# ahmad12hamdan99/CarMPC

Hardware: NVIDIA B200
Metric: terminal-set samples/s (higher is better)
Workload: dtype f64

## Files before the change

### carmpc_b200/_capi.py

```python
from __future__ import annotations

import ctypes
import os

from . import build as _build


class CarmpcError(RuntimeError):
    """A C-ABI call returned a negative status."""


class QPOpts(ctypes.Structure):
    _fields_ = [("rho", ctypes.c_double), ("alpha", ctypes.c_double), ("eps_abs", ctypes.c_double),
                ("eps_rel", ctypes.c_double), ("eps_prim_inf", ctypes.c_double),
                ("max_iter", ctypes.c_int32), ("check_every", ctypes.c_int32),
                ("scaling_iters", ctypes.c_int32), ("polish", ctypes.c_int32)]


class DisturbanceModel(ctypes.Structure):
    _fields_ = [("Bd", ctypes.c_double * 4), ("Cd", ctypes.c_double * 3), ("L1", ctypes.c_double * 12),
                ("L2", ctypes.c_double * 3), ("Bd_plant", ctypes.c_double * 4), ("Cd_plant", ctypes.c_double * 3)]


class LoopNoiseParams(ctypes.Structure):
    _fields_ = [("seed", ctypes.c_uint64), ("first_run", ctypes.c_int64), ("Lw", ctypes.c_double * 16),
                ("Lv", ctypes.c_double * 16)]


_vp, _dp, _i64, _i32 = ctypes.c_void_p, ctypes.c_void_p, ctypes.c_int64, ctypes.c_int

SIGNATURES = {
    "carmpc_last_error": (ctypes.c_char_p, []),
    "carmpc_version": (ctypes.c_char_p, []),
    "carmpc_destroy": (None, [_vp]),
    "carmpc_polytope_create": (_i32, [_dp, _i32, ctypes.POINTER(_vp)]),
    "carmpc_membership_bitset": (_i32, [_vp, _dp, _dp, _dp, _dp, _i64, _vp, _vp, _i32, _vp]),
    "carmpc_polytope_tune": (_i32, [_vp, _dp, _dp, _dp, _dp, _i64, _vp]),
    "carmpc_membership_grid": (_i32, [_vp, _dp, ctypes.POINTER(ctypes.c_int32), ctypes.POINTER(ctypes.c_int32),
                                      _vp, _vp, _vp]),
    "carmpc_membership_bitset_host": (_i32, [_vp, _dp, _dp, _dp, _dp, _i64, _vp, ctypes.POINTER(_i64), _i32]),
    "carmpc_rollout_create": (_i32, [_dp, _dp, _dp, _i32, _dp, _dp, _i32, _dp, _i32, _i32, ctypes.POINTER(_vp)]),
    "carmpc_rollout_bitset": (_i32, [_vp, _dp, _dp, _dp, _dp, _i64, _vp, _vp, _vp, _vp]),
    "carmpc_rollout_bitset_host": (_i32, [_vp, _dp, _dp, _dp, _dp, _i64, _vp, _vp, ctypes.POINTER(_i64)]),
    "carmpc_rollout_get_rows": (_i32, [_vp, _dp, _i32]),
    "carmpc_rollout_reduce_screen": (_i32, [_vp, ctypes.POINTER(ctypes.c_int32), _i32, ctypes.POINTER(ctypes.c_int32), _dp, _i32]),
    "carmpc_scan_staging": (_i32, [_vp, _i32, _i32, _i32]),
    "carmpc_shard_create": (_i32, [_i32, _i32, _i64, ctypes.POINTER(_vp)]),
    "carmpc_shard_export": (_i32, [_vp, _vp]),
    "carmpc_shard_connect": (_i32, [_vp, _vp]),
    "carmpc_shard_connect_local": (_i32, [_vp, ctypes.POINTER(_vp)]),
    "carmpc_membership_bitset_sharded": (_i32, [_vp, _vp, _dp, _dp, _dp, _dp, _i64, _i64, _i64, _i32, _vp, _i32, _vp]),
    "carmpc_rollout_bitset_sharded": (_i32, [_vp, _vp, _dp, _dp, _dp, _dp, _i64, _i64, _i64, _vp, _i32, _vp]),
# ... 73 lines not shown
```

### carmpc_b200/batch.py

```python
from __future__ import annotations

import ctypes
from dataclasses import dataclass
from typing import Optional

import numpy as np

from . import _capi
from ._capi import CarmpcError, check


def _torch():
    import torch
    return torch


def _f64(a) -> np.ndarray:
    return np.ascontiguousarray(a, dtype=np.float64)


def _stream_ptr(stream=None):
    torch = _torch()
    s = torch.cuda.current_stream() if stream is None else stream
    return ctypes.c_void_p(s.cuda_stream)
# ... 11 lines not shown
    def close(self):
        if getattr(self, "_h", None) is not None and self._h:
            self._lib.carmpc_destroy(self._h)
            self._h = ctypes.c_void_p()

    def __del__(self):
        try:
            self.close()
        except Exception:
            pass


class _ScanTuning:
    def set_staging(self, threads_per_cta: int = 256, ring_slots: int = 3, tiles_per_slot: int = 1) -> None:
        check(self._lib.carmpc_scan_staging(self._h, int(threads_per_cta), int(ring_slots), int(tiles_per_slot)))


def _check_soa(x, y, psi, v):
    torch = _torch()
    n = x.numel()
    for t in (x, y, psi, v):
        if not (t.is_cuda and t.dtype == torch.float64 and t.is_contiguous() and t.numel() == n):
            raise ValueError("x, y, psi, v must be contiguous float64 CUDA tensors of equal length")
    return n


class TerminalSetEvaluator(_Handle, _ScanTuning):

    def __init__(self, A: np.ndarray, b: Optional[np.ndarray] = None):
        super().__init__()
# ... 12 lines not shown
    def contains_bits(self, x, y, psi, v, mode: int = 1, bits=None, count=None, stream=None):
        torch = _torch()
        n = _check_soa(x, y, psi, v)
        if bits is None:
            bits = torch.empty((n + 31) // 32, dtype=torch.int32, device=x.device)
        if count is None:
            count = torch.empty(1, dtype=torch.int64, device=x.device)
        check(self._lib.carmpc_membership_bitset(self._h, x.data_ptr(), y.data_ptr(), psi.data_ptr(), v.data_ptr(),
                                                 n, bits.data_ptr(), count.data_ptr(), mode, _stream_ptr(stream)))
        return bits, count

    def tune(self, x, y, psi, v, stream=None) -> None:
        n = _check_soa(x, y, psi, v)
        check(self._lib.carmpc_polytope_tune(self._h, x.data_ptr(), y.data_ptr(), psi.data_ptr(), v.data_ptr(), n,
                                             _stream_ptr(stream)))

    def contains_grid_bits(self, axes, axis_to_state=(0, 1, 2, 3), bits=None, count=None, stream=None):
        torch = _torch()
        axes = [_f64(a).ravel() for a in axes]
        dims = (ctypes.c_int32 * 4)(*[len(a) for a in axes])
        a2s = (ctypes.c_int32 * 4)(*axis_to_state)
        n = int(np.prod([len(a) for a in axes]))
        cat = np.ascontiguousarray(np.concatenate(axes))
        if bits is None:
            bits = torch.empty((n + 31) // 32, dtype=torch.int32, device="cuda")
        if count is None:
            count = torch.empty(1, dtype=torch.int64, device="cuda")
        check(self._lib.carmpc_membership_grid(self._h, _capi.ptr(cat), dims, a2s, bits.data_ptr(), count.data_ptr(),
                                               _stream_ptr(stream)))
        return bits, count
# ... 453 lines not shown
```

### carmpc_b200/csrc/membership.cu

```cuda
#include <math.h>
#include <stdlib.h>

#include <algorithm>
#include <vector>

#include "common.cuh"
#include "shard.cuh"

namespace carmpc {

constexpr int kMaxRows = 512;
constexpr int kThreads = 256;
constexpr int kNS = 4;
constexpr int kChunk = kThreads * kNS;

struct __align__(16) RowF32 {
    float na0, na1, na2, na3;
    float b, pad0, pad1, pad2;
};

struct Staging {
    int threads = 128, stages = 2, tps = 1;
};

// ... 38 lines not shown
        }
        return CARMPC_OK;
    }
    ~HostStage() {
        for (int i = 0; i < 2; ++i) {
            cudaFree(d_coord[i]);
            cudaFree(d_bits[i]);
            cudaFree(d_first[i]);
            if (streams[i]) cudaStreamDestroy(streams[i]);
        }
        cudaFree(d_count);
        cudaFree(d_work);
    }
};

struct Polytope : HandleBase {
    int rows = 0;
    double* d_rows = nullptr;
    RowF32* d_rows32 = nullptr;
    float beta0 = 0.f, beta1 = 0.f;
    HostStage stage;
    std::vector<double> h_rows;
    bool tuned = false;
    Staging staging;
    unsigned long long* d_work = nullptr;
    double* d_axes = nullptr;
    double* h_axes = nullptr;
    ~Polytope() override {
        cudaFree(d_rows);
        cudaFree(d_rows32);
        cudaFree(d_axes);
        cudaFreeHost(h_axes);
        cudaFree(d_work);
    }
};

struct Rollout : HandleBase {
    int s = 0, rin = 0, k_steps = 0, input_mode = 0;
    double* d_data = nullptr;
    RowF32* d_rows32 = nullptr;
    int rows_padded = 0, rows32 = 0;
    float beta0 = 0.f, beta1 = 0.f;
    float in0 = 0.f, in1 = 0.f;
    std::vector<double> h_rows64;
    std::vector<RowF32> h_rows32;
// ... 419 lines not shown
        for (int d = 0; d < kMaxPeers; ++d)
            if (d < sink.n) sink.dst[d][w0] = acc;
        group = __shfl_sync(0xffffffffu, pg, 0);
    }
    block_count<THREADS>(members, count);
    if (tid == 0) {
        __threadfence();
        if (atomicAdd(work + 1, 1ull) == (unsigned long long)gridDim.x - 1ull) {
            work[0] = 0ull;
            work[1] = 0ull;
            __threadfence();
        }
    }
}

struct GridDesc {
    int32_t dims[4];
    int32_t state_of_axis[4];
    int32_t offset[4];
};

__global__ void __launch_bounds__(kThreads, 4)
membership_grid_kernel(const double* __restrict__ g_rows, const RowF32* __restrict__ g_rows32, int rows, int rows_padded,
                       const ScreenConst sc, const double* __restrict__ g_axes, GridDesc gd, int64_t n,
                       uint32_t* __restrict__ bits, unsigned long long* __restrict__ count) {
    extern __shared__ __align__(16) unsigned char smem_raw[];
    double* s_rows = reinterpret_cast<double*>(smem_raw);
    RowF32* s_rows32 = reinterpret_cast<RowF32*>(s_rows + ((rows * 5 + 1) & ~1));
    double* s_axes = reinterpret_cast<double*>(s_rows32 + rows_padded);
    const int axes_len = gd.offset[3] + gd.dims[3];
// ... 205 lines not shown
    dev &= 63;
    if (per_sm_cached[dev] <= 0 || smem_cached[dev] != smem) {
        CARMPC_CUDA(cudaFuncSetAttribute(kernel, cudaFuncAttributeMaxDynamicSharedMemorySize, (int)smem));
        int per_sm = 0;
        CARMPC_CUDA(cudaOccupancyMaxActiveBlocksPerMultiprocessor(&per_sm, kernel, THREADS, smem));
        per_sm_cached[dev] = per_sm > 0 ? per_sm : 1;
        smem_cached[dev] = smem;
    }
    const int64_t n_units = (n_groups + THREADS / 32 - 1) / (THREADS / 32);
    kernel<<<grid_blocks(n_units, per_sm_cached[dev]), THREADS, smem, st>>>(d_exact, d_rows32, es, rows_padded, sc, x, y, p, v,
                                                                      n_groups, sink, count, work);
    CARMPC_CUDA(cudaGetLastError());
    return CARMPC_OK;
}

template <int KIND>
static int launch_scan(const double* d_exact, const RowF32* d_rows32, const ExactSpec es, int rows_padded,
                       const ScreenConst sc, const double* x, const double* y, const double* p, const double* v,
                       int64_t n, BitSink sink, unsigned long long* count, unsigned long long* work, int mode, const Staging& geo,
                       cudaStream_t st) {
    if (n == 0) return CARMPC_OK;
    const bool vec = ((reinterpret_cast<uintptr_t>(x) | reinterpret_cast<uintptr_t>(y) |
                       reinterpret_cast<uintptr_t>(p) | reinterpret_cast<uintptr_t>(v)) & 15) == 0;
    if (vec && mode == 1 && n >= 64 * (int64_t)kChunk) {
        const int64_t n_groups = n / kGroup;
        const size_t smem = scan_tma_smem(es.len, rows_padded, geo);
        int rc = CARMPC_ERR_UNSUPPORTED;
#define TMA_CASE(T, S, P)                                                                                              \
        if (geo.threads == T && geo.stages == S && geo.tps == P)                                                           \
            rc = launch_tma<KIND, T, S, P>(d_exact, d_rows32, es, rows_padded, sc, x, y, p, v, n_groups, sink, count, work, smem, st)
        TMA_CASE(256, 3, 1); TMA_CASE(128, 3, 1); TMA_CASE(128, 4, 1); TMA_CASE(128, 2, 2);
        TMA_CASE(128, 3, 2); TMA_CASE(256, 2, 1); TMA_CASE(128, 2, 1); TMA_CASE(256, 2, 2);
#undef TMA_CASE
        if (rc == CARMPC_ERR_UNSUPPORTED) set_error("membership scan: staging geometry %d/%d/%d is not built", geo.threads, geo.stages, geo.tps);
        if (rc != CARMPC_OK) return rc;
        const int64_t done = n_groups * kGroup;
        if (done == n) return CARMPC_OK;
        x += done; y += done; p += done; v += done; n -= done;
        sink = offset_sink(sink, n_groups);
    }
    const size_t smem = scan_smem(es.len, rows_padded);
    const int64_t n_chunks = (n + kChunk - 1) / kChunk;
#define LAUNCH(M, V)                                                                                              \
    do {                                                                                                          \
        int per_sm = 0;                                                                                           \
        CARMPC_CUDA(cudaOccupancyMaxActiveBlocksPerMultiprocessor(&per_sm, membership_kernel<M, V, KIND>, kThreads, smem)); \
        const int blocks = grid_blocks(n_chunks, per_sm > 0 ? per_sm : 1);                                        \
        membership_kernel<M, V, KIND><<<blocks, kThreads, smem, st>>>(d_exact, d_rows32, es, rows_padded, sc, x, y, p, v, \
// ... 3 lines not shown
        if (vec) LAUNCH(0, true); else LAUNCH(0, false);
    } else {
        if (vec) LAUNCH(1, true); else LAUNCH(1, false);
    }
#undef LAUNCH
    CARMPC_CUDA(cudaGetLastError());
    return CARMPC_OK;
}

static int launch_membership(Polytope* P, const double* x, const double* y, const double* p, const double* v,
                             int64_t n, const BitSink& sink, unsigned long long* count, unsigned long long* work, int mode,
                             cudaStream_t st) {
    ExactSpec es{};
    es.len = P->rows * 5;
    es.rows = P->rows;
    return launch_scan<0>(P->d_rows, P->d_rows32, es, pad_rows(P->rows), screen_const(P), x, y, p, v, n, sink, count, work, mode,
                          P->staging, st);
}

static int launch_rollout(Rollout* R, const double* x, const double* y, const double* p, const double* v, int64_t n,
                          const BitSink& sink, int32_t* first, unsigned long long* count, unsigned long long* work, cudaStream_t st) {
    if (n == 0) return CARMPC_OK;
    if (first == nullptr && R->d_rows32 != nullptr) {
        ExactSpec es{};
        es.len = 20 + 5 * R->s + 5 * R->rin;
        es.s = R->s; es.rin = R->rin; es.k_steps = R->k_steps; es.input_mode = R->input_mode;
        ScreenConst sc;
        sc.beta0 = R->beta0; sc.beta1 = R->beta1; sc.in0 = R->in0; sc.in1 = R->in1;
        return launch_scan<1>(R->d_data, R->d_rows32, es, R->rows_padded, sc, x, y, p, v, n, sink, count, work, 1, R->staging, st);
    }
// ... 104 lines not shown
        if (best < 0 || cnt[best] == 0) break;
        used[best] = 1;
        order.push_back(best);
        size_t w = 0;
        for (unsigned long long m : alive) if (!((m >> best) & 1ull)) alive[w++] = m;
        alive.resize(w);
    }
    for (int r = 0; r < rows; ++r) if (!used[r]) order.push_back(r);
    std::vector<double> sorted(5 * rows);
    for (int i = 0; i < rows; ++i)
        for (int k = 0; k < 5; ++k) sorted[5 * i + k] = P->h_rows[5 * order[i] + k];
    P->h_rows.swap(sorted);
    return upload_rows(P, st);
}

__global__ void __launch_bounds__(256)
pilot32_kernel(const RowF32* __restrict__ g_rows32, int rows, int words, const double* __restrict__ gx,
               const double* __restrict__ gy, const double* __restrict__ gp, const double* __restrict__ gv, int64_t n,
               int64_t stride, int n_sub, unsigned long long* __restrict__ masks) {
    const int k = blockIdx.x * blockDim.x + threadIdx.x;
    if (k >= n_sub) return;
    const int64_t i = (int64_t)k * stride;
    unsigned long long* out = masks + (size_t)k * words;
    for (int w = 0; w < words; ++w) out[w] = 0ull;
    if (i >= n) return;
    const float x = (float)gx[i], y = (float)gy[i], p = (float)gp[i], v = (float)gv[i];
    for (int r = 0; r < rows; ++r) {
        const RowF32 q = g_rows32[r];
        const float m = fmaf(q.na3, v, fmaf(q.na2, p, fmaf(q.na1, y, fmaf(q.na0, x, q.b))));
        if (!(m >= 0.f)) out[r >> 6] |= 1ull << (r & 63);
// ... 98 lines not shown
    }
    const double u8 = 8.0 * 5.9604644775390625e-08, tiny = 1.401298464324817e-45;
    const double b0 = u8 * bmax * 1.000001 + l1max * tiny + 1e-37, b1 = u8 * l1max * 1.000001 + 1e-37;
    if (faithful && b0 < 1e30 && b1 < 1e30) {
        P->beta0 = nextafterf((float)b0, INFINITY);
        P->beta1 = nextafterf((float)b1, INFINITY);
    } else {
        P->beta0 = P->beta1 = INFINITY;
    }
    P->h_rows = sorted;
    h_Ab = sorted.data();
    auto fail = [&](int code) { delete P; return code; };
    if (cudaMalloc(&P->d_rows, sizeof(double) * 5 * (rows > 0 ? rows : 1)) != cudaSuccess ||
        cudaMalloc(&P->d_rows32, sizeof(RowF32) * r32.size()) != cudaSuccess ||
        cudaMalloc(&P->d_work, sizeof(unsigned long long) * 2) != cudaSuccess ||
        cudaMemset(P->d_work, 0, sizeof(unsigned long long) * 2) != cudaSuccess) {
        set_error("carmpc_polytope_create: cudaMalloc failed: %s", cudaGetErrorString(cudaGetLastError()));
        return fail(CARMPC_ERR_CUDA);
    }
    if (rows > 0) {
        if (cudaMemcpy(P->d_rows, h_Ab, sizeof(double) * 5 * rows, cudaMemcpyHostToDevice) != cudaSuccess ||
            cudaMemcpy(P->d_rows32, r32.data(), sizeof(RowF32) * r32.size(), cudaMemcpyHostToDevice) != cudaSuccess) {
            set_error("carmpc_polytope_create: cudaMemcpy failed: %s", cudaGetErrorString(cudaGetLastError()));
            return fail(CARMPC_ERR_CUDA);
        }
    }
    *handle = P;
    return CARMPC_OK;
}

int carmpc_membership_bitset(void* polytope, const double* d_x, const double* d_y, const double* d_psi,
                             const double* d_v, int64_t n, uint32_t* d_bits, int64_t* d_count, int mode,
                             void* stream) {
    Polytope* P = check_handle<Polytope>(polytope, kPolytope);
    CARMPC_REQUIRE(P != nullptr, "not a polytope handle");
    CARMPC_REQUIRE(n >= 0, "n");
    CARMPC_REQUIRE(mode == 0 || mode == 1, "mode must be 0 or 1");
    if (n == 0) {
        if (d_count) CARMPC_CUDA(cudaMemsetAsync(d_count, 0, sizeof(int64_t), (cudaStream_t)stream));
        return CARMPC_OK;
    }
    CARMPC_REQUIRE(d_x && d_y && d_psi && d_v && d_bits, "null device pointer");
    cudaStream_t st = (cudaStream_t)stream;
    if (!P->tuned && n >= ((int64_t)1 << 20)) {
        const int rc = tune_row_order(P, d_x, d_y, d_psi, d_v, n, st);
        if (rc != CARMPC_OK) return rc;
    }
    if (d_count) CARMPC_CUDA(cudaMemsetAsync(d_count, 0, sizeof(int64_t), st));
    return launch_membership(P, d_x, d_y, d_psi, d_v, n, single_sink(d_bits), reinterpret_cast<unsigned long long*>(d_count),
                             P->d_work, mode, st);
}

int carmpc_polytope_tune(void* polytope, const double* d_x, const double* d_y, const double* d_psi, const double* d_v,
                         int64_t n, void* stream) {
    Polytope* P = check_handle<Polytope>(polytope, kPolytope);
    CARMPC_REQUIRE(P != nullptr, "not a polytope handle");
    CARMPC_REQUIRE(n >= 0, "n");
    if (n == 0) return CARMPC_OK;
    CARMPC_REQUIRE(d_x && d_y && d_psi && d_v, "null device pointer");
    return tune_row_order(P, d_x, d_y, d_psi, d_v, n, (cudaStream_t)stream);
}

int carmpc_membership_grid(void* polytope, const double* h_axes, const int32_t dims[4],
                           const int32_t axis_to_state[4], uint32_t* d_bits, int64_t* d_count, void* stream) {
    Polytope* P = check_handle<Polytope>(polytope, kPolytope);
    CARMPC_REQUIRE(P != nullptr, "not a polytope handle");
    CARMPC_REQUIRE(h_axes && dims && axis_to_state && d_bits, "null pointer");
    GridDesc gd;
    int64_t n = 1;
    int off = 0, seen = 0;
    for (int k = 0; k < 4; ++k) {
        CARMPC_REQUIRE(dims[k] >= 1 && dims[k] <= 4096, "each axis must have 1..4096 points");
        CARMPC_REQUIRE(axis_to_state[k] >= 0 && axis_to_state[k] < 4, "axis_to_state entries must be 0..3");
        seen |= 1 << axis_to_state[k];
        gd.dims[k] = dims[k];
// ... 297 lines not shown
                                     const double* d_v, int64_t n_local, int64_t first_sample, int64_t group_stride, int mode,
                                     int64_t* d_total_count, int defer_wait, void* stream) {
    Polytope* P = check_handle<Polytope>(polytope, kPolytope);
    CARMPC_REQUIRE(P != nullptr, "not a polytope handle");
    ShardWindow* W = check_handle<ShardWindow>(shard, kShard);
    CARMPC_REQUIRE(W != nullptr, "not a shard window");
    CARMPC_REQUIRE(mode == 0 || mode == 1, "mode must be 0 or 1");
    CARMPC_REQUIRE(n_local == 0 || (d_x && d_y && d_psi && d_v), "null device pointer");
    BitSink sink{};
    unsigned long long step = 0;
    int rc = shard_sink(W, n_local, first_sample, group_stride, &sink, &step);
    if (rc != CARMPC_OK) return rc;
    cudaStream_t st = (cudaStream_t)stream;
    if (!P->tuned && n_local >= ((int64_t)1 << 20)) {
        rc = tune_row_order(P, d_x, d_y, d_psi, d_v, n_local, st);
        if (rc != CARMPC_OK) return rc;
    }
    rc = launch_membership(P, d_x, d_y, d_psi, d_v, n_local, sink, W->d_local_count, W->d_local_count + 1, mode, st);
    if (rc != CARMPC_OK) return rc;
    CARMPC_REQUIRE(!W->pending, "the previous step of this window was published but never waited for (carmpc_shard_wait)");
    rc = shard_publish_launch(W, st);
    if (rc != CARMPC_OK) return rc;
    if (!defer_wait) {
        rc = shard_wait_launch(W, d_total_count, st);
        if (rc != CARMPC_OK) return rc;
    }
    W->step = step;
    return CARMPC_OK;
}

// ... 45 lines not shown
```

### include/carmpc.h

```cpp
#ifndef CARMPC_H
#define CARMPC_H

#include <stdint.h>

#ifdef __cplusplus
extern "C" {
#endif

typedef enum carmpc_status {
    CARMPC_OK = 0,
    CARMPC_ERR_INVALID = -1,
    CARMPC_ERR_CUDA = -2,
    CARMPC_ERR_NUMERIC = -3,
    CARMPC_ERR_UNSUPPORTED = -4
} carmpc_status;

#define CARMPC_QP_SOLVED 0
#define CARMPC_QP_INFEASIBLE 1
#define CARMPC_QP_MAX_ITER 2

const char* carmpc_last_error(void);
const char* carmpc_version(void);
void carmpc_destroy(void* handle);


int carmpc_polytope_create(const double* h_Ab, int rows, void** handle);

int carmpc_membership_bitset(void* polytope, const double* d_x, const double* d_y, const double* d_psi,
                             const double* d_v, int64_t n, uint32_t* d_bits, int64_t* d_count, int mode,
                             void* stream);

int carmpc_polytope_tune(void* polytope, const double* d_x, const double* d_y, const double* d_psi, const double* d_v,
                         int64_t n, void* stream);

int carmpc_membership_grid(void* polytope, const double* h_axes, const int32_t dims[4],
                           const int32_t axis_to_state[4], uint32_t* d_bits, int64_t* d_count, void* stream);

int carmpc_membership_bitset_host(void* polytope, const double* h_x, const double* h_y, const double* h_psi,
                                  const double* h_v, int64_t n, uint32_t* h_bits, int64_t* h_count, int mode);

int carmpc_rollout_create(const double* h_Ak, const double* h_Acon, const double* h_bcon, int s,
                          const double* h_Ain, const double* h_bin, int rin, const double* h_goal,
                          int k_steps, int input_check_mode, void** handle);

int carmpc_rollout_get_rows(void* rollout, double* h_rows, int capacity);
int carmpc_rollout_reduce_screen(void* rollout, const int32_t* h_kept, int n_kept, const int32_t* h_dual_idx,
                                 const double* h_dual_w, int n_dual);

// ... 131 lines not shown
```

Before: 201.0 billion.

## Add column-subset prefilter stage that skips loading remaining columns for rejected tiles

Adds a two-stage membership kernel. The first stage loads only a subset of the state columns (1 or 3 columns) and uses a conservative bound to reject tiles that lie outside the polytope. The remaining columns are bulk-loaded only for tiles that have survivors. The column subset and row order are chosen at tune time from a pilot sample gathered on the host. The aim is to cut global memory bytes per sample on a bandwidth-bound scan, at the cost of a second dependent load, extra tuning work, and a serial warp-level pipeline.

```diff
diff --git a/carmpc_b200/_capi.py b/carmpc_b200/_capi.py
--- a/carmpc_b200/_capi.py
+++ b/carmpc_b200/_capi.py
@@ -36,6 +36,10 @@
     "carmpc_polytope_create": (_i32, [_dp, _i32, ctypes.POINTER(_vp)]),
     "carmpc_membership_bitset": (_i32, [_vp, _dp, _dp, _dp, _dp, _i64, _vp, _vp, _i32, _vp]),
     "carmpc_polytope_tune": (_i32, [_vp, _dp, _dp, _dp, _dp, _i64, _vp]),
+    "carmpc_polytope_prefilter": (_i32, [_vp, ctypes.POINTER(ctypes.c_int32), ctypes.POINTER(ctypes.c_int32),
+                                         ctypes.POINTER(ctypes.c_double), ctypes.POINTER(_i64)]),
+    "carmpc_prefilter_host": (_i32, [_dp, _i32] + [_dp] * 4 + [_i64] + [_dp] * 4 + [_i64, _vp,
+                                     ctypes.POINTER(ctypes.c_int32), ctypes.POINTER(ctypes.c_double)]),
     "carmpc_membership_grid": (_i32, [_vp, _dp, ctypes.POINTER(ctypes.c_int32), ctypes.POINTER(ctypes.c_int32),
                                       _vp, _vp, _vp]),
     "carmpc_membership_bitset_host": (_i32, [_vp, _dp, _dp, _dp, _dp, _i64, _vp, ctypes.POINTER(_i64), _i32]),
diff --git a/carmpc_b200/batch.py b/carmpc_b200/batch.py
--- a/carmpc_b200/batch.py
+++ b/carmpc_b200/batch.py
@@ -49,6 +49,21 @@
 class _ScanTuning:
     def set_staging(self, threads_per_cta: int = 256, ring_slots: int = 3, tiles_per_slot: int = 1) -> None:
         check(self._lib.carmpc_scan_staging(self._h, int(threads_per_cta), int(ring_slots), int(tiles_per_slot)))
+
+
+def prefilter_host(Ab, pilot, samples):
+    Ab = np.ascontiguousarray(_f64(Ab).reshape(-1, 5))
+    pilot = [np.ascontiguousarray(_f64(a).ravel()) for a in pilot]
+    samples = [np.ascontiguousarray(_f64(a).ravel()) for a in samples]
+    n_pilot, n = len(pilot[0]), len(samples[0])
+    if any(len(a) != n_pilot for a in pilot) or any(len(a) != n for a in samples):
+        raise ValueError("pilot and sample columns must have equal lengths")
+    out = np.zeros(max(n, 1), dtype=np.uint8)
+    info = (ctypes.c_int32 * 2)()
+    bps = ctypes.c_double(0.0)
+    check(_capi.load().carmpc_prefilter_host(_capi.ptr(Ab), len(Ab), *[_capi.ptr(a) for a in pilot], n_pilot,
+                                             *[_capi.ptr(a) for a in samples], n, _capi.ptr(out), info, ctypes.byref(bps)))
+    return out[:n].astype(bool), {"cols": info[0], "rows": info[1], "bytes_per_sample": bps.value}
 
 
 def _check_soa(x, y, psi, v):
@@ -91,6 +106,13 @@
         n = _check_soa(x, y, psi, v)
         check(self._lib.carmpc_polytope_tune(self._h, x.data_ptr(), y.data_ptr(), psi.data_ptr(), v.data_ptr(), n,
                                              _stream_ptr(stream)))
+
+    def prefilter(self) -> dict:
+        cols, rows, loads = ctypes.c_int32(0), ctypes.c_int32(0), ctypes.c_int64(0)
+        bps = ctypes.c_double(0.0)
+        check(self._lib.carmpc_polytope_prefilter(self._h, ctypes.byref(cols), ctypes.byref(rows), ctypes.byref(bps),
+                                                  ctypes.byref(loads)))
+        return {"cols": cols.value, "rows": rows.value, "bytes_per_sample": bps.value, "second_load_tiles": loads.value}
 
     def contains_grid_bits(self, axes, axis_to_state=(0, 1, 2, 3), bits=None, count=None, stream=None):
         torch = _torch()
diff --git a/carmpc_b200/csrc/membership.cu b/carmpc_b200/csrc/membership.cu
--- a/carmpc_b200/csrc/membership.cu
+++ b/carmpc_b200/csrc/membership.cu
@@ -76,6 +76,14 @@
     }
 };
 
+struct Prefilter {
+    int cols = 15;
+    int rows = 0;
+    std::vector<RowF32> r32;
+    float beta0 = INFINITY, beta1 = INFINITY;
+    double bytes = 32.125;
+};
+
 struct Polytope : HandleBase {
     int rows = 0;
     double* d_rows = nullptr;
@@ -88,9 +96,14 @@
     unsigned long long* d_work = nullptr;
     double* d_axes = nullptr;
     double* h_axes = nullptr;
+    Prefilter pre;
+    RowF32* d_rows1 = nullptr;
+    unsigned long long* d_loads = nullptr;
     ~Polytope() override {
         cudaFree(d_rows);
         cudaFree(d_rows32);
+        cudaFree(d_rows1);
+        cudaFree(d_loads);
         cudaFree(d_axes);
         cudaFreeHost(h_axes);
         cudaFree(d_work);
@@ -540,6 +553,278 @@
     }
 }
 
+constexpr int kSplitCols[] = {1, 3};
+
+struct SplitSpec {
+    int cols;
+    int rows_padded;
+    float beta0, beta1;
+};
+
+__host__ __device__ constexpr int col_pos(int cols, int k) {
+    return ((cols >> k) & 1) ? __builtin_popcount(cols & ((1 << k) - 1)) : __builtin_popcount(~cols & ((1 << k) - 1));
+}
+
+template <int COLS>
+__device__ __forceinline__ void stage1(const RowF32* __restrict__ s_rows1, int rows_padded, float beta0, float beta1,
+                                       const float (&c)[4][kNS], bool (&alive)[kNS]) {
+    float nbeta[kNS], mmin[kNS];
+#pragma unroll
+    for (int k = 0; k < kNS; ++k) {
+        float psum = 0.f;
+#pragma unroll
+        for (int q = 0; q < 4; ++q)
+            if ((COLS >> q) & 1) psum += fabsf(c[q][k]);
+        nbeta[k] = -fmaf(beta1, psum, beta0);
+        mmin[k] = kScreenMaxBound;
+    }
+    f32x2 c2[4][kNS / 2];
+#pragma unroll
+    for (int q = 0; q < 4; ++q)
+#pragma unroll
+        for (int k = 0; k < kNS / 2; ++k) c2[q][k] = pack2(c[q][2 * k], c[q][2 * k + 1]);
+    for (int r0 = 0; r0 < rows_padded; r0 += kRowBlock) {
+        bool all_out = true;
+#pragma unroll
+        for (int k = 0; k < kNS; ++k) all_out &= mmin[k] < nbeta[k];
+        if (__all_sync(0xffffffffu, all_out)) break;
+#pragma unroll
+        for (int r = 0; r < kRowBlock; ++r) {
+            const RowF32 q = s_rows1[r0 + r];
+            const float na[4] = {q.na0, q.na1, q.na2, q.na3};
+#pragma unroll
+            for (int k = 0; k < kNS / 2; ++k) {
+                f32x2 m2 = pack2(q.b, q.b);
+#pragma unroll
+                for (int col = 0; col < 4; ++col)
+                    if ((COLS >> col) & 1) m2 = ffma2(pack2(na[col], na[col]), c2[col][k], m2);
+                float m_lo, m_hi;
+                unpack2(m2, m_lo, m_hi);
+                mmin[2 * k] = fminf(mmin[2 * k], m_lo);
+                mmin[2 * k + 1] = fminf(mmin[2 * k + 1], m_hi);
+            }
+        }
+    }
+#pragma unroll
+    for (int k = 0; k < kNS; ++k) alive[k] = !(mmin[k] < nbeta[k] && nbeta[k] >= -kScreenMaxBound);
+}
+
+template <int COLS, int THREADS, int STAGES, int TPS>
+__global__ void __launch_bounds__(THREADS)
+membership_split_kernel(const double* __restrict__ g_rows, const RowF32* __restrict__ g_rows32, const ExactSpec es, int rows_padded,
+                        const ScreenConst sc, const RowF32* __restrict__ g_rows1, const SplitSpec spl,
+                        const double* __restrict__ gx, const double* __restrict__ gy, const double* __restrict__ gp,
+                        const double* __restrict__ gv, int64_t n_groups, const BitSink sink,
+                        unsigned long long* __restrict__ count, unsigned long long* __restrict__ work,
+                        unsigned long long* __restrict__ loads) {
+    extern __shared__ __align__(128) unsigned char smem_raw[];
+    constexpr int kWarps = THREADS / 32;
+    constexpr int kSlot = TPS * kTile;
+    constexpr int kSlotsPerGroup = kGroupTiles / TPS;
+    constexpr uint32_t kArrayBytes = kSlot * sizeof(double);
+    constexpr int n1 = __builtin_popcount(COLS), n2 = 4 - n1;
+    static_assert(kGroupTiles % TPS == 0 && STAGES <= kSlotsPerGroup, "ring geometry");
+    static_assert(COLS > 0 && COLS < 15, "a first stage reads some columns, not all");
+    double* s_ring1 = reinterpret_cast<double*>(smem_raw);
+    double* s_ring2 = s_ring1 + (size_t)kWarps * STAGES * n1 * kSlot;
+    uint64_t* s_bar = reinterpret_cast<uint64_t*>(s_ring2 + (size_t)kWarps * 2 * n2 * kSlot);
+    double* s_rows = reinterpret_cast<double*>(s_bar + kWarps * (STAGES + 2));
+    RowF32* s_rows32 = reinterpret_cast<RowF32*>(s_rows + ((es.len + 1) & ~1));
+    RowF32* s_rows1 = s_rows32 + rows_padded;
+    const int tid = threadIdx.x, warp = tid >> 5, lane = tid & 31;
+    const double* src[4] = {gx, gy, gp, gv};
+    double* w_ring1 = s_ring1 + (size_t)warp * STAGES * n1 * kSlot;
+    double* w_ring2 = s_ring2 + (size_t)warp * 2 * n2 * kSlot;
+    uint64_t* w_bar1 = s_bar + warp * (STAGES + 2);
+    uint64_t* w_bar2 = w_bar1 + STAGES;
+
+    if (lane == 0) {
+        for (int s = 0; s < STAGES + 2; ++s) mbar_init(w_bar1 + s, 1);
+        asm volatile("fence.mbarrier_init.release.cluster;" ::: "memory");
+        asm volatile("fence.proxy.async.shared::cta;" ::: "memory");
+    }
+    stage_rows(g_rows, g_rows32, es.len, rows_padded, s_rows, s_rows32);
+    for (int i = tid; i < spl.rows_padded; i += THREADS) s_rows1[i] = g_rows1[i];
+    __syncthreads();
+
+    int64_t pg = 0;
+    int ps = 0, pj = 0;
+    auto advance = [&]() {
+        if (pg >= n_groups) return;
+        const int64_t sample = pg * kGroup + (int64_t)ps * kSlot;
+        const int stage = pj % STAGES;
+        mbar_expect_tx(w_bar1 + stage, n1 * kArrayBytes);
+#pragma unroll
+        for (int k = 0; k < 4; ++k)
+            if ((COLS >> k) & 1)
+                bulk_load(w_ring1 + ((size_t)stage * n1 + col_pos(COLS, k)) * kSlot, src[k] + sample, kArrayBytes, w_bar1 + stage);
+        ++pj;
+        if (++ps == kSlotsPerGroup) { ps = 0; pg = (int64_t)atomicAdd(work, 1ull); }
+    };
+    if (lane == 0) pg = (int64_t)atomicAdd(work, 1ull);
+    int64_t group = __shfl_sync(0xffffffffu, pg, 0);
+    if (lane == 0)
+        for (int s = 0; s < STAGES; ++s) advance();
+
+    float pf[4][TPS][kNS];
+    bool palive[TPS][kNS];
+    bool pending = false;
+    int64_t pgroup = 0;
+    int ptile = 0;
+    uint32_t r2 = 0, pr = 0;
+    uint32_t acc = 0, acc_old = 0;
+    bool old_waiting = false;
+    int members = 0, second = 0;
+    const int64_t slot_off = sink_slot_offset(sink);
+    auto store_group = [&](int64_t g, uint32_t word) {
+        const int64_t w0 = slot_off + g * sink.stride * (kGroup / 32) + lane;
+#pragma unroll
+        for (int d = 0; d < kMaxPeers; ++d)
+            if (d < sink.n) sink.dst[d][w0] = word;
+    };
+    auto finish = [&]() {
+        const uint32_t q = pr & 1u;
+        mbar_wait(w_bar2 + q, (pr >> 1) & 1u);
+        const double* st2 = w_ring2 + (size_t)q * n2 * kSlot;
+#pragma unroll
+        for (int t = 0; t < TPS; ++t) {
+            float c[4][kNS];
+#pragma unroll
+            for (int col = 0; col < 4; ++col) {
+                if ((COLS >> col) & 1) {
+#pragma unroll
+                    for (int k = 0; k < kNS; ++k) c[col][k] = pf[col][t][k];
+                } else {
+                    const double* a = st2 + (size_t)col_pos(COLS, col) * kSlot + t * kTile + kNS * lane;
+                    const double2 lo = *reinterpret_cast<const double2*>(a), hi = *reinterpret_cast<const double2*>(a + 2);
+                    c[col][0] = (float)lo.x; c[col][1] = (float)lo.y; c[col][2] = (float)hi.x; c[col][3] = (float)hi.y;
+                }
+            }
+            bool in[kNS], amb[kNS];
+#pragma unroll
+            for (int k = 0; k < kNS; ++k) in[k] = palive[t][k];
+            screen32(s_rows32, rows_padded, sc, c[0], c[1], c[2], c[3], in, amb);
+            bool any_amb = false;
+#pragma unroll
+            for (int k = 0; k < kNS; ++k) any_amb |= amb[k];
+            if (__any_sync(0xffffffffu, any_amb)) {
+                const int64_t i0 = pgroup * kGroup + (int64_t)(ptile + t) * kTile + kNS * (int64_t)lane, nn = n_groups * kGroup;
+                double x2[kNS], y2[kNS], p2[kNS], v2[kNS];
+                load4<true>(gx, i0, nn, x2); load4<true>(gy, i0, nn, y2); load4<true>(gp, i0, nn, p2); load4<true>(gv, i0, nn, v2);
+                decide_exact<0>(s_rows, es, x2, y2, p2, v2, amb);
+#pragma unroll
+                for (int k = 0; k < kNS; ++k) in[k] |= amb[k];
+            }
+            const uint32_t word = tile_word(in, members);
+            if ((lane >> 2) == ptile + t) {
+                if (pgroup == group) acc = word;
+                else acc_old = word;
+            }
+        }
+        pending = false;
+        if (pgroup != group && old_waiting) {
+            store_group(pgroup, acc_old);
+            old_waiting = false;
+        }
+    };
+
+    int j = 0;
+    while (group < n_groups) {
+#pragma unroll 1
+        for (int sg = 0; sg < kSlotsPerGroup; ++sg, ++j) {
+            const int stage = j % STAGES;
+            mbar_wait(w_bar1 + stage, (uint32_t)(j / STAGES) & 1u);
+            float f[4][TPS][kNS];
+#pragma unroll
+            for (int t = 0; t < TPS; ++t)
+#pragma unroll
+                for (int col = 0; col < 4; ++col) {
+                    if ((COLS >> col) & 1) {
+                        const double* a = w_ring1 + ((size_t)stage * n1 + col_pos(COLS, col)) * kSlot + t * kTile + kNS * lane;
+                        const double2 lo = *reinterpret_cast<const double2*>(a), hi = *reinterpret_cast<const double2*>(a + 2);
+                        f[col][t][0] = (float)lo.x; f[col][t][1] = (float)lo.y; f[col][t][2] = (float)hi.x; f[col][t][3] = (float)hi.y;
+                    } else {
+#pragma unroll
+                        for (int k = 0; k < kNS; ++k) f[col][t][k] = 0.f;
+                    }
+                }
+            __syncwarp();
+            if (lane == 0) advance();
+            bool alive[TPS][kNS];
+            bool any = false;
+#pragma unroll
+            for (int t = 0; t < TPS; ++t) {
+                float ct[4][kNS];
+#pragma unroll
+                for (int col = 0; col < 4; ++col)
+#pragma unroll
+                    for (int k = 0; k < kNS; ++k) ct[col][k] = f[col][t][k];
+                stage1<COLS>(s_rows1, spl.rows_padded, spl.beta0, spl.beta1, ct, alive[t]);
+#pragma unroll
+                for (int k = 0; k < kNS; ++k) any |= alive[t][k];
+            }
+            const bool survivors = __any_sync(0xffffffffu, any);
+            const uint32_t my_r = r2;
+            if (survivors) {
+                if (lane == 0) {
+                    const uint32_t q = my_r & 1u;
+                    const int64_t sample = group * kGroup + (int64_t)sg * kSlot;
+                    mbar_expect_tx(w_bar2 + q, n2 * kArrayBytes);
+#pragma unroll
+                    for (int k = 0; k < 4; ++k)
+                        if (!((COLS >> k) & 1))
+                            bulk_load(w_ring2 + ((size_t)q * n2 + col_pos(COLS, k)) * kSlot, src[k] + sample, kArrayBytes, w_bar2 + q);
+                }
+                ++r2;
+                ++second;
+            }
+            if (pending) finish();
+            if (survivors) {
+#pragma unroll
+                for (int t = 0; t < TPS; ++t)
+#pragma unroll
+                    for (int k = 0; k < kNS; ++k) {
+                        palive[t][k] = alive[t][k];
+#pragma unroll
+                        for (int col = 0; col < 4; ++col)
+                            if ((COLS >> col) & 1) pf[col][t][k] = f[col][t][k];
+                    }
+                pending = true;
+                pr = my_r;
+                pgroup = group;
+                ptile = sg * TPS;
+            }
+        }
+        if (pending) {
+            acc_old = acc;
+            old_waiting = true;
+        } else {
+            store_group(group, acc);
+        }
+        acc = 0;
+        group = __shfl_sync(0xffffffffu, pg, 0);
+    }
+    if (pending) finish();
+    block_count<THREADS>(members, count);
+    if (tid == 0) {
+        __threadfence();
+        if (atomicAdd(work + 1, 1ull) == (unsigned long long)gridDim.x - 1ull) {
+            work[0] = 0ull;
+            work[1] = 0ull;
+            __threadfence();
+        }
+    }
+    __shared__ int s_second[kWarps];
+    if (lane == 0) s_second[warp] = second;
+    __syncthreads();
+    if (tid == 0 && loads != nullptr) {
+        int total = 0;
+#pragma unroll
+        for (int w = 0; w < kWarps; ++w) total += s_second[w];
+        if (total) atomicAdd(loads, (unsigned long long)total * TPS);
+    }
+}
+
 struct GridDesc {
     int32_t dims[4];
     int32_t state_of_axis[4];
@@ -775,24 +1060,61 @@
     return CARMPC_OK;
 }
 
+static size_t scan_split_smem(int exact_len, int rows_padded, const Staging& g, const SplitSpec& spl) {
+    const int n1 = __builtin_popcount(spl.cols);
+    return sizeof(double) * (g.threads / 32) * (g.stages * n1 + 2 * (4 - n1)) * g.tps * kTile +
+           sizeof(uint64_t) * (g.threads / 32) * (g.stages + 2) + scan_smem(exact_len, rows_padded) +
+           sizeof(RowF32) * spl.rows_padded + 16;
+}
+
+template <int COLS, int THREADS, int STAGES, int TPS>
+static int launch_split(const double* d_exact, const RowF32* d_rows32, const ExactSpec& es, int rows_padded, const ScreenConst& sc,
+                        const RowF32* d_rows1, const SplitSpec& spl, const double* x, const double* y, const double* p,
+                        const double* v, int64_t n_groups, const BitSink& sink, unsigned long long* count,
+                        unsigned long long* work, unsigned long long* loads, size_t smem, cudaStream_t st) {
+    auto kernel = membership_split_kernel<COLS, THREADS, STAGES, TPS>;
+    int per_sm = 0;
+    const int rc = kernel_config((const void*)kernel, THREADS, smem, &per_sm);
+    if (rc != CARMPC_OK) return rc;
+    const int64_t n_units = (n_groups + THREADS / 32 - 1) / (THREADS / 32);
+    kernel<<<grid_blocks(n_units, per_sm > 0 ? per_sm : 1), THREADS, smem, st>>>(d_exact, d_rows32, es, rows_padded, sc, d_rows1,
+                                                                                 spl, x, y, p, v, n_groups, sink, count, work, loads);
+    CARMPC_CUDA(cudaGetLastError());
+    return CARMPC_OK;
+}
+
 template <int KIND>
 static int launch_scan(const double* d_exact, const RowF32* d_rows32, const ExactSpec es, int rows_padded,
                        const ScreenConst sc, const double* x, const double* y, const double* p, const double* v,
                        int64_t n, BitSink sink, unsigned long long* count, unsigned long long* work, int mode, const Staging& geo,
-                       cudaStream_t st) {
+                       cudaStream_t st, const RowF32* d_rows1 = nullptr, const SplitSpec* spl = nullptr,
+                       unsigned long long* loads = nullptr) {
     if (n == 0) return CARMPC_OK;
     const bool vec = ((reinterpret_cast<uintptr_t>(x) | reinterpret_cast<uintptr_t>(y) |
                        reinterpret_cast<uintptr_t>(p) | reinterpret_cast<uintptr_t>(v)) & 15) == 0;
     if (vec && mode == 1 && n >= 64 * (int64_t)kChunk) {
         const int64_t n_groups = n / kGroup;
-        const size_t smem = scan_tma_smem(es.len, rows_padded, geo);
         int rc = CARMPC_ERR_UNSUPPORTED;
+        if (spl == nullptr) {
+            const size_t smem = scan_tma_smem(es.len, rows_padded, geo);
 #define TMA_CASE(T, S, P)                                                                                              \
-        if (geo.threads == T && geo.stages == S && geo.tps == P)                                                           \
-            rc = launch_tma<KIND, T, S, P>(d_exact, d_rows32, es, rows_padded, sc, x, y, p, v, n_groups, sink, count, work, smem, st)
-        TMA_CASE(256, 3, 1); TMA_CASE(128, 3, 1); TMA_CASE(128, 4, 1); TMA_CASE(128, 2, 2);
-        TMA_CASE(128, 3, 2); TMA_CASE(256, 2, 1); TMA_CASE(128, 2, 1); TMA_CASE(256, 2, 2);
+            if (geo.threads == T && geo.stages == S && geo.tps == P)                                                       \
+                rc = launch_tma<KIND, T, S, P>(d_exact, d_rows32, es, rows_padded, sc, x, y, p, v, n_groups, sink, count, work, smem, st)
+            TMA_CASE(256, 3, 1); TMA_CASE(128, 3, 1); TMA_CASE(128, 4, 1); TMA_CASE(128, 2, 2);
+            TMA_CASE(128, 3, 2); TMA_CASE(256, 2, 1); TMA_CASE(128, 2, 1); TMA_CASE(256, 2, 2);
 #undef TMA_CASE
+        } else if (KIND == 0) {
+            const size_t smem = scan_split_smem(es.len, rows_padded, geo, *spl);
+#define SPLIT_CASE(T, S, P)                                                                                            \
+            if (geo.threads == T && geo.stages == S && geo.tps == P)                                                       \
+                rc = spl->cols == 1 ? launch_split<1, T, S, P>(d_exact, d_rows32, es, rows_padded, sc, d_rows1, *spl, x, y, p, v,   \
+                                                              n_groups, sink, count, work, loads, smem, st)                      \
+                                    : launch_split<3, T, S, P>(d_exact, d_rows32, es, rows_padded, sc, d_rows1, *spl, x, y, p, v,   \
+                                                              n_groups, sink, count, work, loads, smem, st)
+            SPLIT_CASE(256, 3, 1); SPLIT_CASE(128, 3, 1); SPLIT_CASE(128, 4, 1); SPLIT_CASE(128, 2, 2);
+            SPLIT_CASE(128, 3, 2); SPLIT_CASE(256, 2, 1); SPLIT_CASE(128, 2, 1); SPLIT_CASE(256, 2, 2);
+#undef SPLIT_CASE
+        }
         if (rc == CARMPC_ERR_UNSUPPORTED) set_error("membership scan: staging geometry %d/%d/%d is not built", geo.threads, geo.stages, geo.tps);
         if (rc != CARMPC_OK) return rc;
         const int64_t done = n_groups * kGroup;
@@ -826,6 +1148,15 @@
     ExactSpec es{};
     es.len = P->rows * 5;
     es.rows = P->rows;
+    if (P->pre.cols != 15 && mode == 1) {
+        SplitSpec spl;
+        spl.cols = P->pre.cols;
+        spl.rows_padded = (int)P->pre.r32.size();
+        spl.beta0 = P->pre.beta0;
+        spl.beta1 = P->pre.beta1;
+        return launch_scan<0>(P->d_rows, P->d_rows32, es, pad_rows(P->rows), screen_const(P), x, y, p, v, n, sink, count, work,
+                              mode, P->staging, st, P->d_rows1, &spl, P->d_loads);
+    }
     return launch_scan<0>(P->d_rows, P->d_rows32, es, pad_rows(P->rows), screen_const(P), x, y, p, v, n, sink, count, work, mode,
                           P->staging, st);
 }
@@ -960,6 +1291,182 @@
     return upload_rows(P, st);
 }
 
+static void column_box(const double* rows, int n, double lo[4], double hi[4]) {
+    for (int k = 0; k < 4; ++k) { lo[k] = -INFINITY; hi[k] = INFINITY; }
+    for (int r = 0; r < n; ++r) {
+        const double* a = rows + 5 * r;
+        int nz = 0, k = 0;
+        for (int c = 0; c < 4; ++c)
+            if (a[c] != 0.0) { ++nz; k = c; }
+        if (nz != 1 || !std::isfinite(a[4])) continue;
+        const long double b = a[4];
+        const long double q = (b + fabsl(b) * 0x1p-50L + 0x1p-1070L) / (long double)a[k];
+        const long double w = fabsl(q) * 0x1p-40L;
+        if (a[k] > 0) hi[k] = std::min(hi[k], nextafter((double)(q + w), INFINITY));
+        else lo[k] = std::max(lo[k], nextafter((double)(q - w), -INFINITY));
+    }
+}
+
+static bool fold_rows(const double* rows, int n, int cols, const double lo[4], const double hi[4], Prefilter& F) {
+    F = Prefilter();
+    F.cols = cols;
+    long double bmax = 0, l1max = 0;
+    for (int r = 0; r < n; ++r) {
+        const double* a = rows + 5 * r;
+        bool touches = false;
+        for (int c = 0; c < 4; ++c) touches = touches || (((cols >> c) & 1) && a[c] != 0.0);
+        if (!touches || a[4] == INFINITY) continue;
+        if (!std::isfinite(a[4])) return false;
+        long double fold = a[4], mag = fabsl((long double)a[4]), l1 = 0;
+        for (int c = 0; c < 4; ++c) {
+            if ((cols >> c) & 1) { l1 += fabsl((long double)a[c]); continue; }
+            if (a[c] == 0.0) continue;
+            const long double al = (long double)a[c] * lo[c], ah = (long double)a[c] * hi[c];
+            const long double m = fabsl((long double)a[c]) * std::max(fabsl((long double)lo[c]), fabsl((long double)hi[c]));
+            fold += m * 0x1p-50L - std::min(al, ah);
+            mag += m;
+        }
+        fold += mag * 0x1p-40L + 0x1p-1070L;
+        const double bd = nextafter((double)fold, INFINITY);
+        RowF32 q;
+        q.na0 = (cols & 1) ? (float)-a[0] : 0.f; q.na1 = (cols & 2) ? (float)-a[1] : 0.f;
+        q.na2 = (cols & 4) ? (float)-a[2] : 0.f; q.na3 = (cols & 8) ? (float)-a[3] : 0.f;
+        q.b = (float)bd;
+        q.pad0 = q.pad1 = q.pad2 = 0.f;
+        if (!(std::isfinite(q.na0) && std::isfinite(q.na1) && std::isfinite(q.na2) && std::isfinite(q.na3) && std::isfinite(q.b)))
+            return false;
+        F.r32.push_back(q);
+        bmax = std::max(bmax, (long double)fabs(bd));
+        l1max = std::max(l1max, l1);
+    }
+    if (F.r32.empty()) return false;
+    const long double u8 = 8.0L * 5.9604644775390625e-08L, tiny = 1.401298464324817e-45L;
+    const long double b0 = u8 * bmax * 1.000001L + l1max * tiny + 1e-37L, b1 = u8 * l1max * 1.000001L + l1max * 0x1p-50L + 1e-37L;
+    if (!(b0 < 1e30L && b1 < 1e30L)) return false;
+    F.beta0 = nextafterf((float)b0, INFINITY);
+    F.beta1 = nextafterf((float)b1, INFINITY);
+    F.rows = (int)F.r32.size();
+    return true;
+}
+
+static bool stage1_survives(const Prefilter& F, const float (&c)[4], unsigned long long* mask) {
+    float psum = 0.f;
+    for (int k = 0; k < 4; ++k)
+        if ((F.cols >> k) & 1) psum += fabsf(c[k]);
+    const float nbeta = -fmaf(F.beta1, psum, F.beta0);
+    float mmin = kScreenMaxBound;
+    for (int r = 0; r < F.rows; ++r) {
+        const RowF32& q = F.r32[r];
+        const float na[4] = {q.na0, q.na1, q.na2, q.na3};
+        float m = q.b;
+        for (int k = 0; k < 4; ++k)
+            if ((F.cols >> k) & 1) m = fmaf(na[k], c[k], m);
+        mmin = fminf(mmin, m);
+        if (mask != nullptr && m < nbeta) *mask |= 1ull << r;
+        if (mask == nullptr && mmin < nbeta) break;
+    }
+    return !(mmin < nbeta && nbeta >= -kScreenMaxBound);
+}
+
+static void stage1_coords(int cols, const double* const pts[4], int64_t i, float (&c)[4]) {
+    for (int k = 0; k < 4; ++k) c[k] = ((cols >> k) & 1) ? (float)pts[k][i] : 0.f;
+}
+
+static Prefilter build_prefilter(const double* rows, int n, const double* const pilot[4], int64_t n_pilot) {
+    Prefilter best;
+    const int64_t tiles = n_pilot / kTile;
+    if (n < 1 || n > 64 || tiles < 1) return best;
+    double lo[4], hi[4];
+    column_box(rows, n, lo, hi);
+    int need = 0;
+    for (int k = 0; k < 4; ++k)
+        if (!(std::isfinite(lo[k]) && std::isfinite(hi[k]))) need |= 1 << k;
+    double best_bytes = 0.9 * 32.125;
+    for (int cols : kSplitCols) {
+        if ((cols & need) != need) continue;
+        Prefilter F;
+        if (!fold_rows(rows, n, cols, lo, hi, F)) continue;
+        int64_t survived = 0;
+        for (int64_t t = 0; t < tiles; ++t) {
+            for (int i = 0; i < kTile; ++i) {
+                float c[4];
+                stage1_coords(cols, pilot, t * kTile + i, c);
+                if (stage1_survives(F, c, nullptr)) { ++survived; break; }
+            }
+        }
+        const int n1 = __builtin_popcount(cols);
+        F.bytes = 8.0 * n1 + 8.0 * (4 - n1) * (double)survived / (double)tiles + 0.125;
+        if (F.bytes < best_bytes) { best_bytes = F.bytes; best = F; }
+    }
+    if (best.cols == 15) return best;
+    std::vector<unsigned long long> alive;
+    for (int64_t i = 0; i < tiles * kTile; ++i) {
+        float c[4];
+        stage1_coords(best.cols, pilot, i, c);
+        unsigned long long m = 0ull;
+        stage1_survives(best, c, &m);
+        if (m) alive.push_back(m);
+    }
+    std::vector<int> order;
+    std::vector<char> used(best.rows, 0);
+    while (!alive.empty()) {
+        int cnt[64] = {0};
+        for (unsigned long long m : alive)
+            for (unsigned long long t = m; t; t &= t - 1) ++cnt[__builtin_ctzll(t)];
+        int pick = -1;
+        for (int r = 0; r < best.rows; ++r) if (!used[r] && (pick < 0 || cnt[r] > cnt[pick])) pick = r;
+        if (pick < 0 || cnt[pick] == 0) break;
+        used[pick] = 1;
+        order.push_back(pick);
+        size_t w = 0;
+        for (unsigned long long m : alive) if (!((m >> pick) & 1ull)) alive[w++] = m;
+        alive.resize(w);
+    }
+    for (int r = 0; r < best.rows; ++r) if (!used[r]) order.push_back(r);
+    std::vector<RowF32> sorted(pad_rows(best.rows));
+    for (RowF32& q : sorted) { q.na0 = q.na1 = q.na2 = q.na3 = 0.f; q.b = INFINITY; q.pad0 = q.pad1 = q.pad2 = 0.f; }
+    for (int i = 0; i < best.rows; ++i) sorted[i] = best.r32[order[i]];
+    best.r32.swap(sorted);
+    return best;
+}
+
+__global__ void __launch_bounds__(kTile)
+gather_tiles_kernel(const double* __restrict__ gx, const double* __restrict__ gy, const double* __restrict__ gp,
+                    const double* __restrict__ gv, int64_t n_tiles, int picks, double* __restrict__ out) {
+    const int64_t tile = (int64_t)blockIdx.x * n_tiles / picks;
+    const double* src[4] = {gx, gy, gp, gv};
+#pragma unroll
+    for (int a = 0; a < 4; ++a) out[((size_t)a * picks + blockIdx.x) * kTile + threadIdx.x] = src[a][tile * kTile + threadIdx.x];
+}
+
+static int tune_prefilter(Polytope* P, const double* x, const double* y, const double* p, const double* v, int64_t n,
+                          cudaStream_t st) {
+    const int64_t n_tiles = n / kTile;
+    if (P->rows < 1 || P->rows > 64 || n_tiles < 1) return CARMPC_OK;
+    const int picks = (int)std::min<int64_t>(512, n_tiles);
+    double* d_tiles = nullptr;
+    CARMPC_CUDA(cudaMalloc(&d_tiles, sizeof(double) * 4 * kTile * picks));
+    gather_tiles_kernel<<<picks, kTile, 0, st>>>(x, y, p, v, n_tiles, picks, d_tiles);
+    std::vector<double> h((size_t)4 * kTile * picks);
+    cudaError_t err = cudaGetLastError();
+    if (err == cudaSuccess) err = cudaMemcpyAsync(h.data(), d_tiles, sizeof(double) * h.size(), cudaMemcpyDeviceToHost, st);
+    if (err == cudaSuccess) err = cudaStreamSynchronize(st);
+    cudaFree(d_tiles);
+    CARMPC_CUDA(err);
+    const double* pilot[4];
+    for (int a = 0; a < 4; ++a) pilot[a] = h.data() + (size_t)a * kTile * picks;
+    Prefilter F = build_prefilter(P->h_rows.data(), P->rows, pilot, (int64_t)kTile * picks);
+    if (F.cols != 15) {
+        cudaFree(P->d_rows1);
+        P->d_rows1 = nullptr;
+        CARMPC_CUDA(cudaMalloc(&P->d_rows1, sizeof(RowF32) * F.r32.size()));
+        CARMPC_CUDA(cudaMemcpyAsync(P->d_rows1, F.r32.data(), sizeof(RowF32) * F.r32.size(), cudaMemcpyHostToDevice, st));
+        CARMPC_CUDA(cudaStreamSynchronize(st));
+    }
+    P->pre = F;
+    return CARMPC_OK;
+}
+
 __global__ void __launch_bounds__(256)
 pilot32_kernel(const RowF32* __restrict__ g_rows32, int rows, int words, const double* __restrict__ gx,
                const double* __restrict__ gy, const double* __restrict__ gp, const double* __restrict__ gv, int64_t n,
@@ -1088,7 +1595,9 @@
     if (cudaMalloc(&P->d_rows, sizeof(double) * 5 * (rows > 0 ? rows : 1)) != cudaSuccess ||
         cudaMalloc(&P->d_rows32, sizeof(RowF32) * r32.size()) != cudaSuccess ||
         cudaMalloc(&P->d_work, sizeof(unsigned long long) * 2) != cudaSuccess ||
-        cudaMemset(P->d_work, 0, sizeof(unsigned long long) * 2) != cudaSuccess) {
+        cudaMemset(P->d_work, 0, sizeof(unsigned long long) * 2) != cudaSuccess ||
+        cudaMalloc(&P->d_loads, sizeof(unsigned long long)) != cudaSuccess ||
+        cudaMemset(P->d_loads, 0, sizeof(unsigned long long)) != cudaSuccess) {
         set_error("carmpc_polytope_create: cudaMalloc failed: %s", cudaGetErrorString(cudaGetLastError()));
         return fail(CARMPC_ERR_CUDA);
     }
@@ -1117,7 +1626,8 @@
     CARMPC_REQUIRE(d_x && d_y && d_psi && d_v && d_bits, "null device pointer");
     cudaStream_t st = (cudaStream_t)stream;
     if (!P->tuned && n >= ((int64_t)1 << 20)) {
-        const int rc = tune_row_order(P, d_x, d_y, d_psi, d_v, n, st);
+        int rc = tune_row_order(P, d_x, d_y, d_psi, d_v, n, st);
+        if (rc == CARMPC_OK) rc = tune_prefilter(P, d_x, d_y, d_psi, d_v, n, st);
         if (rc != CARMPC_OK) return rc;
     }
     if (d_count) CARMPC_CUDA(cudaMemsetAsync(d_count, 0, sizeof(int64_t), st));
@@ -1132,7 +1642,45 @@
     CARMPC_REQUIRE(n >= 0, "n");
     if (n == 0) return CARMPC_OK;
     CARMPC_REQUIRE(d_x && d_y && d_psi && d_v, "null device pointer");
-    return tune_row_order(P, d_x, d_y, d_psi, d_v, n, (cudaStream_t)stream);
+    const int rc = tune_row_order(P, d_x, d_y, d_psi, d_v, n, (cudaStream_t)stream);
+    if (rc != CARMPC_OK) return rc;
+    return tune_prefilter(P, d_x, d_y, d_psi, d_v, n, (cudaStream_t)stream);
+}
+
+int carmpc_polytope_prefilter(void* polytope, int32_t* cols, int32_t* stage1_rows, double* bytes_per_sample,
+                              int64_t* second_load_tiles) {
+    Polytope* P = check_handle<Polytope>(polytope, kPolytope);
+    CARMPC_REQUIRE(P != nullptr, "not a polytope handle");
+    if (cols) *cols = P->pre.cols;
+    if (stage1_rows) *stage1_rows = P->pre.rows;
+    if (bytes_per_sample) *bytes_per_sample = P->pre.bytes;
+    if (second_load_tiles) {
+        unsigned long long c = 0;
+        CARMPC_CUDA(cudaMemcpy(&c, P->d_loads, sizeof(c), cudaMemcpyDeviceToHost));
+        *second_load_tiles = (int64_t)c;
+    }
+    return CARMPC_OK;
+}
+
+int carmpc_prefilter_host(const double* h_Ab, int rows, const double* px, const double* py, const double* pp, const double* pv,
+                          int64_t n_pilot, const double* tx, const double* ty, const double* tp, const double* tv, int64_t n,
+                          uint8_t* h_survive, int32_t* info, double* bytes_per_sample) {
+    CARMPC_REQUIRE(h_Ab != nullptr && rows >= 0 && rows <= kMaxRows && n_pilot >= 0 && n >= 0, "rows, n_pilot, n");
+    CARMPC_REQUIRE(n_pilot == 0 || (px && py && pp && pv), "null pilot pointer");
+    CARMPC_REQUIRE(n == 0 || (tx && ty && tp && tv && h_survive), "null sample pointer");
+    for (int i = 0; i < 5 * rows; ++i)
+        CARMPC_REQUIRE(i % 5 == 4 ? !isnan(h_Ab[i]) : std::isfinite(h_Ab[i]), "non-finite coefficient or NaN bound");
+    const double* pilot[4] = {px, py, pp, pv};
+    const Prefilter F = build_prefilter(h_Ab, rows, pilot, n_pilot);
+    const double* pts[4] = {tx, ty, tp, tv};
+    for (int64_t i = 0; i < n; ++i) {
+        float c[4];
+        stage1_coords(F.cols, pts, i, c);
+        h_survive[i] = F.cols == 15 ? 1 : (uint8_t)stage1_survives(F, c, nullptr);
+    }
+    if (info) { info[0] = F.cols; info[1] = F.rows; }
+    if (bytes_per_sample) *bytes_per_sample = F.bytes;
+    return CARMPC_OK;
 }
 
 int carmpc_membership_grid(void* polytope, const double* h_axes, const int32_t dims[4],
@@ -1460,6 +2008,7 @@
     cudaStream_t st = (cudaStream_t)stream;
     if (!P->tuned && n_local >= ((int64_t)1 << 20)) {
         rc = tune_row_order(P, d_x, d_y, d_psi, d_v, n_local, st);
+        if (rc == CARMPC_OK) rc = tune_prefilter(P, d_x, d_y, d_psi, d_v, n_local, st);
         if (rc != CARMPC_OK) return rc;
     }
     rc = launch_membership(P, d_x, d_y, d_psi, d_v, n_local, sink, W->d_local_count, W->d_local_count + 1, mode, st);
diff --git a/include/carmpc.h b/include/carmpc.h
--- a/include/carmpc.h
+++ b/include/carmpc.h
@@ -32,6 +32,13 @@
 
 int carmpc_polytope_tune(void* polytope, const double* d_x, const double* d_y, const double* d_psi, const double* d_v,
                          int64_t n, void* stream);
+
+int carmpc_polytope_prefilter(void* polytope, int32_t* cols, int32_t* stage1_rows, double* bytes_per_sample,
+                              int64_t* second_load_tiles);
+
+int carmpc_prefilter_host(const double* h_Ab, int rows, const double* px, const double* py, const double* ppsi,
+                          const double* pv, int64_t n_pilot, const double* x, const double* y, const double* psi,
+                          const double* v, int64_t n, uint8_t* h_survive, int32_t* info, double* bytes_per_sample);
 
 int carmpc_membership_grid(void* polytope, const double* h_axes, const int32_t dims[4],
                            const int32_t axis_to_state[4], uint32_t* d_bits, int64_t* d_count, void* stream);
```

Measured after the change: 221.8 billion (median of 6 runs). 10.3% higher.
